# yisol/IDM-VTON

Hardware: AMD Instinct MI355X
Metric: try-on images/sec at 768x1024, 30 DDIM steps, guidance 2.0 (higher is better)
Workload: dtype bf16; 1 GPU; BASELINE.json configs[1]: 768x1024, 30 steps, batch 2/GPU, guidance 2.0, bf16 storage / fp32 accumulate, scheduler ddim, hipGraph on, GarmentNet batched over 6 timesteps, GarmentNet(block b+1)||TryonNet(block b) two-stream overlap on; images_per_call=2, parallelism=dp1 (image shards, one start-up RCCL weight broadcast), rccl_ranks=1

## Files before the change

idm-vton_amd/csrc/gemm_body.cuh:

```cuda
#pragma once
#include <type_traits>
#if !defined(__gfx950__) && !defined(__gfx942__) && defined(__HIP_DEVICE_COMPILE__)
#error "gemm_body.cuh: the counted vmcnt pipeline is written for gfx94x/gfx950 (stores counted in vmcnt)"
#endif
#include "common.cuh"
#include "gemm_common.cuh"

template <typename T, int BN, int BM, int WN, int WM, int ST, bool V1, bool LIN, bool PF, bool TR, bool XA = false>
__device__ __forceinline__ void gemm_body(const GemmParams& p, char* smem, const int m0, const int n0) {
    typedef typename VT<T>::v8 v8;
    typedef typename VT<T>::v4 v4;
    constexpr int NW = WN * WM;
    constexpr int SN = BN / WN, SM = BM / WM;
    constexpr int NI = SN / 32, MI = SM / 32;
    constexpr int WBYTES = BN * 128, XBYTES = BM * 128;
    constexpr int PW_ = BN / 8, PX_ = BM / 8;
    constexpr bool UNEVEN = (PW_ % NW != 0) || (PX_ % NW != 0);
    constexpr int WI = (PW_ + NW - 1) / NW, XI = (PX_ + NW - 1) / NW;
    static_assert(BN % 8 == 0 && BM % 8 == 0 && WN * SN == BN && WM * SM == BM && NI * 32 == SN && MI * 32 == SM, "tile / wave-count mismatch");
    static_assert(!UNEVEN || (V1 && ST == 2), "round-robin piece assignment needs the two-stage ring");
    char* sW = smem;
    char* sX = smem + ST * WBYTES;

    const int lane = threadIdx.x & 63;
// ... 110 lines not shown
    for (int ni = 0; ni < NI; ++ni)
#pragma unroll
        for (int mi = 0; mi < MI; ++mi)
#pragma unroll
            for (int r = 0; r < 16; ++r) acc[ni][mi][r] = 0.f;

    auto frag_a = [&](const char* bW, int s, int ni) { return *(const v8*)(bW + a_row[ni] + (((2 * s + u) ^ a_swz[ni]) << 4)); };
    auto frag_b = [&](const char* bX, int s, int mi) { return *(const v8*)(bX + b_row[mi] + (((2 * s + u) ^ b_swz[mi]) << 4)); };
    auto compute = [&](int buf, bool spread = false, int t_next = 0, int buf_next = 0) {
        const char* bW = sW + buf * WBYTES;
        const char* bX = sX + buf * XBYTES;
        if constexpr (!PF) {
#pragma unroll
            for (int s = 0; s < 4; ++s) {
                v8 a[NI], b[MI];
#pragma unroll
                for (int ni = 0; ni < NI; ++ni) a[ni] = frag_a(bW, s, ni);
#pragma unroll
                for (int mi = 0; mi < MI; ++mi) b[mi] = frag_b(bX, s, mi);
                if constexpr (V1) {
                    if (spread) issue_part(t_next, buf_next, s);
                    __builtin_amdgcn_sched_barrier(0);
                }
#pragma unroll
                for (int ni = 0; ni < NI; ++ni)
#pragma unroll
                    for (int mi = 0; mi < MI; ++mi)
                        acc[ni][mi] = TR ? VT<T>::mfma(b[mi], a[ni], acc[ni][mi]) : VT<T>::mfma(a[ni], b[mi], acc[ni][mi]);
            }
        } else {
            v8 a[2][NI], b[2][MI];
#pragma unroll
            for (int ni = 0; ni < NI; ++ni) a[0][ni] = frag_a(bW, 0, ni);
#pragma unroll
            for (int mi = 0; mi < MI; ++mi) b[0][mi] = frag_b(bX, 0, mi);
#pragma unroll
            for (int s = 0; s < 4; ++s) {
                if (s < 3) {
#pragma unroll
                    for (int ni = 0; ni < NI; ++ni) a[(s + 1) & 1][ni] = frag_a(bW, s + 1, ni);
#pragma unroll
                    for (int mi = 0; mi < MI; ++mi) b[(s + 1) & 1][mi] = frag_b(bX, s + 1, mi);
                }
                if (spread) issue_part(t_next, buf_next, s);
                __builtin_amdgcn_sched_barrier(0);
#pragma unroll
                for (int ni = 0; ni < NI; ++ni)
#pragma unroll
                    for (int mi = 0; mi < MI; ++mi)
                        acc[ni][mi] = TR ? VT<T>::mfma(b[s & 1][mi], a[s & 1][ni], acc[ni][mi])
                                         : VT<T>::mfma(a[s & 1][ni], b[s & 1][mi], acc[ni][mi]);
                __builtin_amdgcn_sched_barrier(0);
            }
        }
    };

    v8 xkf[XA ? XA_NK : 1];
    int xa_b = 0, xa_h = 0;
    if constexpr (XA) {
        static_assert(NI == 2 && !TR, "fused cross-attention: one 64-channel head per wave");
        const int mw = m0 + wm * SM;
        xa_b = (mw < p.M ? mw : p.M - 1) / p.xa.tokens;
        xa_h = (n0 + wn * SN) >> 6;
        xattn_load_k<T>(p.xa, xa_b, xa_h, lane, xkf);
    }
    const int nt = p.Ktot >> 6;
    if constexpr (!V1) {
        issue(0, 0);
        for (int t = 0; t < nt; ++t) {
            asm volatile("s_waitcnt vmcnt(0)" ::: "memory");
            __syncthreads();
            if (t + 1 < nt) issue(t + 1, (t + 1) & 1);
            compute(t & 1);
        }
    } else {
        constexpr int LPT = WI + XI;
        static_assert((ST - 2) * LPT < 64, "vmcnt immediate is 6 bits");
#pragma unroll
        for (int s = 0; s < ST - 1; ++s)
            if (s < nt) issue(s, s);
        int cbuf = 0, ibuf = ST - 1;
        for (int t = 0; t < nt; ++t) {
            if (t + ST - 2 < nt) wait_vmcnt<(ST - 2) * LPT>(); else wait_vmcnt<0>();
            __builtin_amdgcn_s_barrier();
            asm volatile("" ::: "memory");
            compute(cbuf, t + ST - 1 < nt, t + ST - 1, ibuf);
            cbuf = cbuf + 1 == ST ? 0 : cbuf + 1;
            ibuf = ibuf + 1 == ST ? 0 : ibuf + 1;
        }
    }

    if constexpr (XA) {
        v8 xvf[XA_NV];
        xattn_load_v<T>(p.xa, xa_b, xa_h, lane, xvf);
        xattn_compute<T, MI>(p.xa, p.M, acc, m0 + wm * SM, lane, xkf, xvf);
    }
    gemm_epilogue<T, NI, MI, SN, SM, TR>(p, acc, m0, n0, wn, wm, lane);
}

template <typename T, int BN, int BM, int WN, int WM, int ST, bool V1, bool LIN, int OCC, bool PFX = false>
__global__ __launch_bounds__(WN * WM * 64, OCC) void gemm_conv_kernel(const GemmParams p) {
    __shared__ __attribute__((aligned(1024))) char smem[ST * (BN + BM) * 128];
    const int wg = xcd_remap(blockIdx.x, p.tiles_m * p.tiles_n);
    int tm, tn;
    if constexpr (!V1) { tm = wg / p.tiles_n; tn = wg - tm * p.tiles_n; }
    else {
        const int GM = p.gm > 0 ? p.gm : 1024 / BM;
        const int width = GM * p.tiles_n;
        const int grp = wg / width, rem = wg - grp * width;
        const int first = grp * GM;
        const int gsz = p.tiles_m - first < GM ? p.tiles_m - first : GM;
        tn = rem / gsz; tm = first + (rem - tn * gsz);
    }
    const int m0 = tm * BM, n0 = tn * BN;
    if constexpr (BN == 320) {
        gemm_body<T, BN, BM, WN, WM, ST, V1, LIN, OCC == 1 || PFX, false>(p, smem, m0, n0);
    } else {
        if (p.vt != nullptr && n0 >= p.vt_n0) gemm_body<T, BN, BM, WN, WM, ST, V1, LIN, OCC == 1 || PFX, true>(p, smem, m0, n0);
        else gemm_body<T, BN, BM, WN, WM, ST, V1, LIN, OCC == 1 || PFX, false>(p, smem, m0, n0);
    }
}

template <typename T, int BN, int BM, int WN, int WM, int ST, int OCC>
__global__ __launch_bounds__(WN * WM * 64, OCC) void gemm_xattn_kernel(const GemmParams p) {
    __shared__ __attribute__((aligned(1024))) char smem[ST * (BN + BM) * 128];
    const int wg = xcd_remap(blockIdx.x, p.tiles_m * p.tiles_n);
    const int GM = p.gm > 0 ? p.gm : 1024 / BM;
    const int width = GM * p.tiles_n;
    const int grp = wg / width, rem = wg - grp * width;
    const int first = grp * GM;
    const int gsz = p.tiles_m - first < GM ? p.tiles_m - first : GM;
    const int tn = rem / gsz, tm = first + (rem - tn * gsz);
    gemm_body<T, BN, BM, WN, WM, ST, true, true, OCC == 1, false, true>(p, smem, tm * BM, tn * BN);
}

template <typename T, int BN, int BM, int WN, int WM, int ST, bool V1, int OCC, bool PFX = false>
static void launch_cfg(const GemmParams& p0, bool lin, hipStream_t st) {
    GemmParams p = p0;
    p.gm = V1 ? idmvton_choose_gm(p.tiles_m, p.tiles_n, BM, BN, p.Ktot) : 0;
    const dim3 grid(p.tiles_n * p.tiles_m), block(WN * WM * 64);
    if constexpr (V1) {
        if (lin) { hipLaunchKernelGGL((gemm_conv_kernel<T, BN, BM, WN, WM, ST, true, true, OCC, PFX>), grid, block, 0, st, p); return; }
    }
    hipLaunchKernelGGL((gemm_conv_kernel<T, BN, BM, WN, WM, ST, V1, false, OCC, PFX>), grid, block, 0, st, p);
}


int gemm_tiles_v0(const GemmParams& p, bool bf16, int bn, int bm, bool lin, hipStream_t st);
int gemm_tiles_v1(const GemmParams& p, bool bf16, int bn, int bm, bool lin, hipStream_t st);
int gemm_tiles_v2(const GemmParams& p, bool bf16, int bn, int bm, bool lin, hipStream_t st);
int gemm_tiles_w8(const GemmParams& p, bool bf16, int bn, int bm, int form, bool lin, hipStream_t st);
int gemm_tiles_xattn(const GemmParams& p, bool bf16, int bn, int bm, int w8, hipStream_t st);
int launch_gemm_lin(const GemmParams& p, bool bf16, int bm, int form, int grid_cap, hipStream_t st);
```

idm-vton_amd/csrc/gemm_conv.hip:

```cpp
#include <cstdlib>
#include <cstring>
#include <vector>
#include "gemm_body.cuh"

int launch_gemm_lin(const GemmParams& p, bool bf16, int bm, int form, int grid_cap, hipStream_t st);

#include <map>
#include <mutex>
#include <tuple>
int idmvton_choose_gm(int tiles_m, int tiles_n, int bm, int bn, int K) {
    static const char* env = getenv("IDMVTON_GM");
    if (env) return atoi(env);
    static const bool model = getenv("IDMVTON_GM_MODEL") && atoi(getenv("IDMVTON_GM_MODEL")) != 0;
    if (!model) return 0;
    static std::mutex mu;
    static std::map<std::tuple<int, int, int, int, int>, int> cache;
    const auto key = std::make_tuple(tiles_m, tiles_n, bm, bn, K);
    std::lock_guard<std::mutex> lk(mu);
    auto it = cache.find(key);
    if (it != cache.end()) return it->second;
    const int T = tiles_m * tiles_n, q = T / 8, r = T % 8;
    static const long cap = getenv("IDMVTON_GM_CAP_KB") ? atol(getenv("IDMVTON_GM_CAP_KB")) << 10 : (2l << 20);
    long best = -1; int best_gm = 0;
    for (int gm = 1; gm <= tiles_m; ++gm) {
        if (gm > 1 && (long)gm * bm * K * 2 > cap) break;
        long cost = 0;
        for (int x = 0; x < 8; ++x) {
            const int lo = x < r ? x * (q + 1) : r * (q + 1) + (x - r) * q, n = x < r ? q + 1 : q;
            int m_lo = tiles_m, m_hi = -1;
            std::vector<char> ms(tiles_m, 0), ns(tiles_n, 0);
            int cm = 0, cn = 0;
            for (int wg = lo; wg < lo + n; ++wg) {
                const int width = gm * tiles_n, grp = wg / width, rem = wg - grp * width, first = grp * gm;
                const int gsz = tiles_m - first < gm ? tiles_m - first : gm;
                const int tn = rem / gsz, tm = first + (rem - tn * gsz);
                if (!ms[tm]) { ms[tm] = 1; ++cm; }
                if (!ns[tn]) { ns[tn] = 1; ++cn; }
            }
            (void)m_lo; (void)m_hi;
            cost += (long)cm * bm + (long)cn * bn;
        }
        if (best < 0 || cost < best) { best = cost; best_gm = gm; }
    }
    cache[key] = best_gm;
    return best_gm;
}

static int launch_gemm(const GemmParams& p0, bool bf16, int variant, int bn, int bm, bool lin, hipStream_t st) {
    GemmParams p = p0;
    int form = 0;
    int grid_cap = 0;
    if (variant == 5) { form = bm & 15; grid_cap = (bm & 0x4000) ? 5 : 0; bm &= ~(15 | 0x4000); }
    p.tiles_n = (p.N + bn - 1) / bn;
    p.tiles_m = (p.M + bm - 1) / bm;
    int rc = 1;
    if (p.mode == IDMVTON_EPI_XATTN) {
        if (bm != 64 && p.xa.tokens % 64 != 0) {
            bm = 64;
            p.tiles_m = (p.M + bm - 1) / bm;
        }
        if (gemm_tiles_xattn(p, bf16, bn, bm, variant == 6 && bn == 128 && bm == 128, st))
            return idmvton_set_error(IDMVTON_E_ARG, "gemm_conv: IDMVTON_EPI_XATTN runs on the 128x64, 128x128 and 128x256 tiles (got %dx%d)", bn, bm);
        CHECK_LAUNCH("gemm_conv");
        return IDMVTON_OK;
    }
    if (variant == 0) rc = gemm_tiles_v0(p, bf16, bn, bm, lin, st);
    else if (variant == 1) rc = gemm_tiles_v1(p, bf16, bn, bm, lin, st);
    else if (variant == 2) rc = gemm_tiles_v2(p, bf16, bn, bm, lin, st);
    else if (variant == 5) {
        if (!(bn == 256 && (bm == 256 || bm == 192))) return idmvton_set_error(IDMVTON_E_ARG, "gemm_conv: variant 5 is the 256x256 / 256x192 tile");
        if (lin) rc = launch_gemm_lin(p, bf16, bm, form, grid_cap, st);
        else if (bm == 256) rc = gemm_tiles_v1(p, bf16, 256, 256, lin, st);
        else {
            p.tiles_n = (p.N + 127) / 128; p.tiles_m = (p.M + 255) / 256;
            rc = gemm_tiles_v1(p, bf16, 128, 256, lin, st);
        }
    } else if (variant == 6) {
        const int form6 = bm & 15;
        bm &= ~15;
        p.tiles_m = (p.M + bm - 1) / bm;
        if (bn == 320 && (p.vt || !p.wide || p.out8 || p.mode == IDMVTON_EPI_GEGLU)) {
            const int fbn = bn == 320 ? 128 : bn, fbm = bn == 320 ? 256 : bm;
            p.tiles_n = (p.N + fbn - 1) / fbn;
            p.tiles_m = (p.M + fbm - 1) / fbm;
            rc = gemm_tiles_v1(p, bf16, fbn, fbm, lin, st);
        } else rc = gemm_tiles_w8(p, bf16, bn, bm, form6, lin, st);
    } else return idmvton_set_error(IDMVTON_E_ARG, "gemm_conv: unknown variant %d", variant);
    if (rc) return idmvton_set_error(IDMVTON_E_ARG, "gemm_conv: variant %d has no %dx%d tile", variant, bn, bm);
    CHECK_LAUNCH("gemm_conv");
    return IDMVTON_OK;
}

extern "C" int idmvton_gemm_conv(const idmvton_gemm_conv_args* a, void* stream) {
    CHECK_ARG(a != nullptr, IDMVTON_E_ARG, "gemm_conv: null args");
    CHECK_ARG(a->dtype == IDMVTON_F16 || a->dtype == IDMVTON_BF16, IDMVTON_E_DTYPE, "gemm_conv: dtype %d", a->dtype);
    CHECK_ARG(a->M > 0 && a->N > 0 && a->Ktot > 0, IDMVTON_E_SHAPE, "gemm_conv: M=%d N=%d K=%d", a->M, a->N, a->Ktot);
    CHECK_ARG(a->Ktot % 64 == 0, IDMVTON_E_SHAPE, "gemm_conv: Ktot=%d must be a multiple of 64", a->Ktot);
    CHECK_ARG(a->N % 4 == 0, IDMVTON_E_SHAPE, "gemm_conv: N=%d must be a multiple of 4", a->N);
    CHECK_ARG(a->nseg >= 1 && a->nseg <= IDMVTON_MAX_SEG, IDMVTON_E_SHAPE, "gemm_conv: nseg=%d", a->nseg);
    int ksum = 0;
    for (int s = 0; s < a->nseg; ++s) {
        const idmvton_seg& g = a->seg[s];
        CHECK_ARG(g.ptr && g.len > 0 && g.len % 64 == 0, IDMVTON_E_SHAPE, "gemm_conv: seg %d len=%d", s, g.len);
        CHECK_ARG(g.pitch % 8 == 0 && g.coff % 8 == 0, IDMVTON_E_ALIGN, "gemm_conv: seg %d pitch=%d coff=%d", s, g.pitch, g.coff);
        CHECK_ARG(g.bytes < 0x80000000u, IDMVTON_E_SHAPE, "gemm_conv: seg %d tensor >= 2 GiB", s);
        CHECK_ARG(((uintptr_t)g.ptr & 15) == 0, IDMVTON_E_ALIGN, "gemm_conv: seg %d pointer not 16-byte aligned", s);
        ksum += g.len;
    }
    CHECK_ARG(ksum == a->Ktot, IDMVTON_E_SHAPE, "gemm_conv: segment lengths sum to %d, Ktot=%d", ksum, a->Ktot);
    CHECK_ARG(a->Ho > 0 && a->Wo > 0 && a->Hi > 0 && a->Wi > 0 && a->stride > 0 && a->M % (a->Ho * a->Wo) == 0,
              IDMVTON_E_SHAPE, "gemm_conv: geometry M=%d Ho=%d Wo=%d", a->M, a->Ho, a->Wo);
    if (a->ups) CHECK_ARG(a->stride == 1 && a->Ho <= 2 * a->Hi && a->Ho >= 2 * a->Hi - 1 && a->Wo <= 2 * a->Wi && a->Wo >= 2 * a->Wi - 1, IDMVTON_E_SHAPE,
                          "gemm_conv: ups=1 needs stride 1 and an output grid of 2Hi x 2Wi or one short of it (Ho=%d Hi=%d Wo=%d Wi=%d)", a->Ho, a->Hi, a->Wo, a->Wi);
    CHECK_ARG(a->w && ((uintptr_t)a->w & 15) == 0, IDMVTON_E_ALIGN, "gemm_conv: weight pointer");
    const uint64_t wbytes = (uint64_t)a->N * a->Ktot * 2;
    CHECK_ARG(wbytes + (uint64_t)128 * a->Ktot * 2 < 0xFFFFFFFFull, IDMVTON_E_SHAPE, "gemm_conv: weight too large");
    const bool geglu = a->mode == IDMVTON_EPI_GEGLU, xattn = a->mode == IDMVTON_EPI_XATTN;
    CHECK_ARG(a->mode == IDMVTON_EPI_NONE || a->mode == IDMVTON_EPI_GELU || a->mode == IDMVTON_EPI_QUICKGELU || geglu || xattn, IDMVTON_E_ARG, "gemm_conv: mode %d", a->mode);
    CHECK_ARG(a->colscale_n >= 0 && a->colscale_n % 4 == 0 && !(geglu && a->colscale_n), IDMVTON_E_ARG, "gemm_conv: colscale_n=%d", a->colscale_n);
    if (geglu) CHECK_ARG(a->N % 64 == 0 && !a->res && !a->rowbias && !a->vt, IDMVTON_E_ARG, "gemm_conv: GEGLU needs N%%64==0, no res/rowbias/vt");
    CHECK_ARG(a->out || (a->vt && a->vt_n0 == 0), IDMVTON_E_ARG, "gemm_conv: null out");
    if (a->out) CHECK_ARG(a->ldo % 4 == 0 && ((uintptr_t)a->out & 7) == 0, IDMVTON_E_ALIGN, "gemm_conv: out alignment");
    if (a->res) CHECK_ARG(a->ldr % 4 == 0 && ((uintptr_t)a->res & 7) == 0, IDMVTON_E_ALIGN, "gemm_conv: res alignment");
    if (a->bias) CHECK_ARG(((uintptr_t)a->bias & 7) == 0, IDMVTON_E_ALIGN, "gemm_conv: bias alignment");
    if (a->rowbias) CHECK_ARG(a->rowbias_ld % 4 == 0 && a->rows_per_group > 0 && ((uintptr_t)a->rowbias & 7) == 0,
                              IDMVTON_E_ALIGN, "gemm_conv: rowbias");
    if (a->vt && a->vt_perm) CHECK_ARG(((uintptr_t)a->vt & 15) == 0, IDMVTON_E_ALIGN, "gemm_conv: vt pointer not 16-byte aligned");
    if (a->vt && a->vt_perm) CHECK_ARG(a->vt_tokens % 16 == 0, IDMVTON_E_ARG, "gemm_conv: vt_perm needs vt_tokens %% 16 == 0 (got %d)", a->vt_tokens);
    if (a->vt) CHECK_ARG(a->vt_tokens > 0 && a->vt_tokens % 4 == 0 && a->M % a->vt_tokens == 0 && a->vt_n0 % 64 == 0 &&
                         a->vt_n0 >= 0 && a->vt_n0 < a->N && ((uintptr_t)a->vt & 7) == 0,
                         IDMVTON_E_ARG, "gemm_conv: vt_tokens=%d vt_n0=%d", a->vt_tokens, a->vt_n0);

    GemmParams p;
    memset(&p.xa, 0, sizeof(p.xa));
    if (xattn) {
        const idmvton_xattn* x = a->xattn;
        CHECK_ARG(x != nullptr && (x->nseg == 1 || x->nseg == 2), IDMVTON_E_ARG, "gemm_conv: IDMVTON_EPI_XATTN needs `xattn` with 1 or 2 key segments");
        CHECK_ARG(a->N % 64 == 0 && !a->bias && !a->res && !a->rowbias && !a->vt && !a->colscale_n && !a->io_flags &&
                  a->nseg == 1 && a->Ho == 1 && a->Hi == 1 && a->Wo == a->M && a->Wi == a->M && a->out && a->ldo % 8 == 0 && ((uintptr_t)a->out & 15) == 0,
                  IDMVTON_E_ARG, "gemm_conv: IDMVTON_EPI_XATTN is a plain Linear with N %% 64 == 0 and nothing else in its epilogue");
        CHECK_ARG(x->tokens > 0 && x->tokens % 32 == 0 && a->M % x->tokens == 0, IDMVTON_E_SHAPE, "gemm_conv: xattn.tokens=%d (rows per batch element, a multiple of 32 dividing M=%d)", x->tokens, a->M);
        for (int s = 0; s < x->nseg; ++s) {
            const int nk_max = s == 0 ? 96 : 32;
            CHECK_ARG(x->k[s] && x->vt[s] && x->nk[s] > 0 && x->nk[s] <= nk_max && x->k_rows[s] >= ((x->nk[s] + 31) & ~31) && x->ldk[s] >= a->N && x->ldk[s] % 8 == 0 &&
                      x->ldvt[s] >= ((x->nk[s] + 15) & ~15) && x->ldvt[s] % 8 == 0 && (((uintptr_t)x->k[s] | (uintptr_t)x->vt[s]) & 15) == 0, IDMVTON_E_SHAPE,
                      "gemm_conv: xattn segment %d: nk=%d (<= %d) k_rows=%d (>= round32(nk)) ldk=%d ldvt=%d (>= round16(nk))", s, x->nk[s], nk_max, x->k_rows[s], x->ldk[s], x->ldvt[s]);
            p.xa.k[s] = x->k[s]; p.xa.vt[s] = x->vt[s]; p.xa.ldk[s] = x->ldk[s]; p.xa.ldvt[s] = x->ldvt[s]; p.xa.nk[s] = x->nk[s]; p.xa.krows[s] = x->k_rows[s];
        }
        p.xa.nseg = x->nseg; p.xa.tokens = x->tokens; p.xa.vchan = a->N; p.xa.ip_scale = x->ip_scale;
    } else CHECK_ARG(a->xattn == nullptr, IDMVTON_E_ARG, "gemm_conv: `xattn` without mode IDMVTON_EPI_XATTN");
    p.w = a->w; p.w_bytes = (uint32_t)wbytes; p.N = a->N; p.Ktot = a->Ktot;
    p.nseg = a->nseg;
    for (int s = 0; s < IDMVTON_MAX_SEG; ++s) p.seg[s] = a->seg[s < a->nseg ? s : a->nseg - 1];
    p.M = a->M; p.Ho = a->Ho; p.Wo = a->Wo; p.Hi = a->Hi; p.Wi = a->Wi; p.stride = a->stride; p.ups = a->ups ? 1 : 0;
    p.out = a->out; p.ldo = a->ldo; p.bias = a->bias; p.rowbias = a->rowbias; p.rowbias_ld = a->rowbias_ld;
    p.rows_per_group = a->rows_per_group > 0 ? a->rows_per_group : 1; p.res = a->res; p.ldr = a->ldr; p.mode = a->mode;
    p.vt = a->vt; p.vt_n0 = a->vt_n0; p.vt_tokens = a->vt_tokens > 0 ? a->vt_tokens : 4; p.vt_perm = a->vt_perm ? 1 : 0;
    p.colscale_n = a->colscale_n; p.colscale = a->colscale;
    p.tiles_m = p.tiles_n = 0; p.gm = 0;
    {
        auto a16 = [](const void* q) { return ((uintptr_t)q & 15) == 0; };
        const int n_out = geglu ? a->N / 2 : a->N;
        p.wide = n_out % 8 == 0 && a->N % 8 == 0 && a->colscale_n % 8 == 0 && (!a->out || (a->ldo % 8 == 0 && a16(a->out))) &&
                 (!a->res || (a->ldr % 8 == 0 && a16(a->res))) && (!a->bias || a16(a->bias)) &&
                 (!a->rowbias || (a->rowbias_ld % 8 == 0 && a16(a->rowbias))) && (!a->vt || a->vt_n0 % 8 == 0);
    }

    int variant = 1, bn = 64, bm = 64;
    static const bool env_narrow = getenv("IDMVTON_EPILOGUE_8B") != nullptr;
    if ((a->tile_hint & 0x8000) || env_narrow) p.wide = 0;
    p.res32 = (a->io_flags & IDMVTON_IO_RES_F32) ? 1 : 0;
    p.out32 = (a->io_flags & IDMVTON_IO_OUT_F32) ? 1 : 0;
    p.bias32 = (a->io_flags & IDMVTON_IO_BIAS_F32) ? 1 : 0;
    if (p.bias32) CHECK_ARG(a->bias && p.wide && !geglu && !a->vt && ((uintptr_t)a->bias & 15) == 0, IDMVTON_E_ARG,
                            "gemm_conv: IDMVTON_IO_BIAS_F32 needs a 16-byte aligned bias and the plain 16-byte epilogue (no GEGLU, no vt)");
    CHECK_ARG((a->io_flags & ~15) == 0, IDMVTON_E_ARG, "gemm_conv: io_flags=%d", a->io_flags);
    p.out8 = (a->io_flags & IDMVTON_IO_OUT_F8) ? 1 : 0;
    p.o8_scale = a->f8_out_scale; p.vt8_scale = a->f8_vt_scale;
    if (p.out8) {
        CHECK_ARG(a->io_flags == IDMVTON_IO_OUT_F8 && a->mode == IDMVTON_EPI_NONE && !a->res && !a->rowbias && p.wide,
                  IDMVTON_E_ARG, "gemm_conv: IDMVTON_IO_OUT_F8 needs the plain 16-byte epilogue (no activation / residual / rowbias / fp32 IO)");
        CHECK_ARG((!a->out || a->f8_out_scale > 0.f) && (!a->vt || (a->f8_vt_scale > 0.f && a->vt_tokens % 64 == 0 && ((uintptr_t)a->vt & 15) == 0)),
                  IDMVTON_E_ARG, "gemm_conv: IDMVTON_IO_OUT_F8: scales > 0, vt_tokens %% 64 == 0 (got %d), 16-byte aligned vt", a->vt_tokens);
    }
    if (p.res32 || p.out32) {
        CHECK_ARG((a->io_flags & ~7) == 0 && !geglu && !a->vt, IDMVTON_E_ARG, "gemm_conv: io_flags=%d (fp32 res / out: no GEGLU, no vt)", a->io_flags);
        CHECK_ARG(!p.res32 || a->res, IDMVTON_E_ARG, "gemm_conv: IDMVTON_IO_RES_F32 without res");
        CHECK_ARG(p.wide, IDMVTON_E_ALIGN, "gemm_conv: the fp32 residual stream needs the 16-byte epilogue (N, ldo, ldr multiples of 8, 16-byte aligned pointers)");
    }
    if (a->tile_hint) { variant = (a->tile_hint >> 28) & 0xf; bn = (a->tile_hint >> 16) & 0xfff; bm = a->tile_hint & 0x7fff; }
    else {
        static const int cand[5][2] = {{256, 256}, {128, 256}, {128, 128}, {128, 64}, {64, 64}};
        for (int i = 0; i < 5; ++i) {
            const int n_ = cand[i][0], m_ = cand[i][1];
            if (geglu && n_ < 128) continue;
            if (xattn && (n_ != 128)) continue;
            if (a->vt && a->vt_n0 % n_ != 0) continue;
            if (i < 4 && (n_ > ((a->N + 63) & ~63) || m_ > ((a->M + 63) & ~63))) continue;
            bn = n_; bm = m_;
            if ((long)((a->N + n_ - 1) / n_) * ((a->M + m_ - 1) / m_) >= 200) break;
        }
    }
    if (geglu) CHECK_ARG(bn >= 128, IDMVTON_E_ARG, "gemm_conv: GEGLU needs BN >= 128 (64-row wave tiles)");
    if (a->vt) CHECK_ARG(a->vt_n0 % bn == 0, IDMVTON_E_ARG, "gemm_conv: vt_n0 %% BN != 0");
    const idmvton_seg& s0 = a->seg[0];
    const bool lin = a->nseg == 1 && a->Ho == 1 && a->Hi == 1 && a->Wo == a->M && a->Wi == a->M && a->stride == 1 &&
                     !a->ups && s0.dy == 0 && s0.dx == 0 && (uint64_t)a->M * s0.pitch * 2 < 0x80000000ull;
    if (!a->tile_hint && bn == 256 && bm == 256 && lin) { variant = 5; bm = 257; }
    else if (!a->tile_hint && !xattn) {
        if (bn == 256 && bm == 256) variant = 6;
        else if (bn == 128 && bm == 128) variant = 6;
        if (a->N > 256 && a->N <= 320 && p.wide && !a->vt && !geglu && !p.out8 && (a->M + 191) / 192 >= 200) { variant = 6; bn = 320; bm = 192; }
    }
    hipStream_t st = (hipStream_t)stream;
    return launch_gemm(p, a->dtype == IDMVTON_BF16, variant, bn, bm, lin, st);
}
```

idm-vton_amd/ops.py:

```python
import ctypes as C
import json
import os

import torch

from . import ffi

_DT = {torch.float16: ffi.F16, torch.bfloat16: ffi.BF16}


def _dt(t):
    try:
        return _DT[t.dtype]
    except KeyError:
        raise TypeError(f"idm_vton_amd ops take float16/bfloat16 tensors, got {t.dtype}") from None


def _stream():
    return torch.cuda.current_stream().cuda_stream


PROFILE = None


def _call(fn_name, args, flops=0.0, bytes_=0.0, seg_nb=None):
    launch = (lambda: ffi.call(fn_name, args, _stream())) if seg_nb is None else (lambda: ffi.call_shared(fn_name, args, seg_nb, _stream()))
    if PROFILE is None:
        launch()
        return
    e0, e1 = torch.cuda.Event(enable_timing=True), torch.cuda.Event(enable_timing=True)
    e0.record()
    launch()
    e1.record()
    PROFILE.append((fn_name, e0, e1, flops, bytes_))


TUNE_PATH = os.environ.get("IDMVTON_TUNE_TABLE") or os.path.join(os.path.dirname(os.path.abspath(__file__)), "tune_gfx950.json")
_TUNE = {"gemm": {}, "attn": {}}
RECORD = None


def load_tune(path=TUNE_PATH):
    global _TUNE
    _TUNE = {"gemm": {}, "attn": {}}
    if path and os.path.exists(path):
        with open(path) as f:
            t = json.load(f)
        _TUNE = {"gemm": dict(t.get("gemm", {})), "attn": dict(t.get("attn", {}))}
        for kind in ("gemm", "attn") if os.environ.get("IDMVTON_TUNE_NO_MIRROR") != "1" else ():
            for k, v in list(_TUNE[kind].items()):
                d, rest = k.split(",", 1)
                if d in ("0", "1"):
                    _TUNE[kind].setdefault(("1" if d == "0" else "0") + "," + rest, v)
    return _TUNE


def gemm_key(a):
    return "%d,%d,%d,%d,%d,%d,%d,%d,%d,%d" % (a.dtype, a.M, a.N, a.Ktot, a.nseg, a.Wo, a.stride, a.ups, a.mode, 1 if a.vt else 0)


def attn_key(a):
    return "%d,%d,%d,%d,%d,%d,%d,%d,%d" % (a.dtype, a.mode, a.B, a.heads, a.Nq, a.nseg, a.nk[0], a.nk[1] if a.nseg > 1 else 0,
                                          a.seg_b0[1] if a.nseg > 1 else 0)


def _dev(t):
    if not t.is_cuda:
        raise RuntimeError("idm_vton_amd ops run on the GPU only (tensor is on %s); there is no CPU fallback" % t.device)
    return t


def _ptr(t):
    return None if t is None else _dev(t).data_ptr()


class SegSpec:
    __slots__ = ("t", "coff", "len", "dy", "dx")

    def __init__(self, t, coff, length, dy=0, dx=0):
        self.t, self.coff, self.len, self.dy, self.dx = t, coff, length, dy, dx


def gemm_conv(segs, w, M, *, Ho=1, Wo=None, Hi=1, Wi=None, stride=1, ups=False, out=None, ldo=None, bias=None,
              rowbias=None, rowbias_ld=0, rows_per_group=1, res=None, ldr=None, geglu=False, gelu=False, quick_gelu=False, vt=None,
              vt_n0=0, vt_tokens=0, vt_perm=True, colscale_n=0, colscale=1.0, tile_hint=0, out_f32=False, xattn=None, f8=None):
    if f8 is not None:
        if res is not None or rowbias is not None or geglu or gelu or quick_gelu or (bias is not None and bias.dtype == torch.float32):
            raise ValueError("gemm_conv(f8=...): no residual / rowbias / activation, and the bias in the storage dtype (not fp32)")
        if vt is not None and vt_tokens % 64 != 0:
            raise ValueError(f"gemm_conv(f8=...): vt_tokens must be a multiple of 64 (got {vt_tokens})")
    a = ffi.GemmConvArgs()
    a.dtype = _dt(w)
    N, Ktot = w.shape
    a.w, a.N, a.Ktot = _ptr(w), N, Ktot
    a.nseg = len(segs)
    for i, s in enumerate(segs):
        t = _dev(s.t)
        g = a.seg[i]
        pitch = t.shape[-1]
        for d in range(t.dim() - 2, -1, -1):
            if t.shape[d] > 1:
                pitch = t.stride(d)
                break
        extent = 1 + sum((n - 1) * st for n, st in zip(t.shape, t.stride()))
        g.ptr, g.bytes, g.pitch = t.data_ptr(), extent * t.element_size(), pitch
        g.coff, g.len, g.dy, g.dx = s.coff, s.len, s.dy, s.dx
    Wo = M if Wo is None else Wo
    Wi = M if Wi is None else Wi
    a.M, a.Ho, a.Wo, a.Hi, a.Wi, a.stride, a.ups = M, Ho, Wo, Hi, Wi, stride, int(bool(ups))
    n_out = N // 2 if geglu else (vt_n0 if vt is not None else N)
    if out is None and n_out > 0:
        out = torch.empty((M, n_out), dtype=torch.uint8 if f8 is not None else (torch.float32 if out_f32 else w.dtype), device=w.device)
    if f8 is not None:
        if (out is not None and out.dtype != torch.uint8) or (vt is not None and vt.dtype != torch.uint8):
            raise TypeError("gemm_conv(f8=...): out / vt must be uint8 (e4m3 bytes)")
        a.f8_out_scale, a.f8_vt_scale = float(f8[0]), float(f8[1])
    a.io_flags = ffi.IO_OUT_F8 if f8 is not None else (
        (ffi.IO_RES_F32 if res is not None and res.dtype == torch.float32 else 0) |
        (ffi.IO_OUT_F32 if out is not None and out.dtype == torch.float32 else 0) |
        (ffi.IO_BIAS_F32 if bias is not None and bias.dtype == torch.float32 else 0))
    a.out = _ptr(out)
    a.ldo = (ldo if ldo is not None else (out.stride(-2) if out is not None else 0))
    a.bias = _ptr(bias)
    a.rowbias, a.rowbias_ld, a.rows_per_group = _ptr(rowbias), rowbias_ld, rows_per_group
    a.res = _ptr(res)
    a.ldr = (ldr if ldr is not None else (res.stride(-2) if res is not None else 0))
    a.mode = ffi.EPI_GEGLU if geglu else (ffi.EPI_GELU if gelu else (ffi.EPI_QUICKGELU if quick_gelu else ffi.EPI_NONE))
    xa, xflops = None, 0.0
    if xattn is not None:
        xa = ffi.XAttn()
        xa.nseg, xa.tokens, xa.ip_scale = len(xattn["segs"]), xattn["tokens"], xattn.get("ip_scale", 1.0)
        for i, sg in enumerate(xattn["segs"]):
            xa.k[i], xa.vt[i], xa.ldk[i], xa.ldvt[i], xa.nk[i], xa.k_rows[i] = _ptr(sg["k"]), _ptr(sg["vt"]), sg["ldk"], sg["ldvt"], sg["nk"], sg["k_rows"]
            xflops += 4.0 * M * N * sg["nk"]
        a.mode, a.xattn = ffi.EPI_XATTN, C.pointer(xa)
    a.vt, a.vt_n0, a.vt_tokens = _ptr(vt), vt_n0, vt_tokens
    a.vt_perm = int(bool(vt_perm)) if vt is not None else 0
    a.colscale_n, a.colscale = colscale_n, colscale
    a.tile_hint = tile_hint if tile_hint else _TUNE["gemm"].get(gemm_key(a), 0)
    if RECORD is not None:
        RECORD.append(("gemm", gemm_key(a), type(a).from_buffer_copy(a), (segs, w, out, bias, rowbias, res, vt, xa, xattn)))
    seen, xbytes = set(), 0
    for sg in segs:
        if sg.t.data_ptr() not in seen:
            seen.add(sg.t.data_ptr())
            xbytes += sg.t.numel() * sg.t.element_size()
    esz = w.element_size()
    obytes = (M * (N // 2 if geglu else N)) * (out.element_size() if out is not None else esz) + (M * N * res.element_size() if res is not None else 0)
    _call("idmvton_gemm_conv", a, flops=2.0 * M * N * Ktot + xflops, bytes_=float(xbytes + N * Ktot * esz + obytes))
    return out


def xattn_q_weight(w):
    return w.index_select(0, key_order_index(w.shape[0], w.device)).contiguous()


def key_order_index(n, device=None):
    if n % 16:
        raise ValueError("key order needs a multiple of 16 keys, got %d" % n)
    i = torch.arange(n, device=device)
    return (i & ~12) | ((i & 4) << 1) | ((i & 8) >> 1)


def key_order(vt):
    return vt.index_select(-1, key_order_index(vt.shape[-1], vt.device)).contiguous()


def round16(n):
    return (n + 15) // 16 * 16


def linear(x, w, **kw):
    M, K = x.shape
    return gemm_conv([SegSpec(x, 0, K)], w, M, **kw)


def conv_segs(x, k, pad, coff=0, length=None):
    length = x.shape[-1] if length is None else length
    return [SegSpec(x, coff, length, ky - pad, kx - pad) for ky in range(k) for kx in range(k)]


QSCALE = 0.125 * 1.4426950408889634


def attention(q, out, segs, heads, *, mode=ffi.ATTN_SELF, ip_scale=1.0, B=None, Nq=None, ldq=None, ldo=None, tune=0, q_prescaled=False):
    a = ffi.AttnArgs()
    a.dtype, a.mode = _dt(q), mode
    a.B = q.shape[0] if B is None else B
    a.Nq = q.shape[1] if Nq is None else Nq
    a.heads = heads
    a.q, a.ldq = _ptr(q), (q.stride(-2) if ldq is None else ldq)
    a.out, a.ldo = _ptr(out), (out.stride(-2) if ldo is None else ldo)
    a.nseg = len(segs)
    for i, s in enumerate(segs):
        a.k[i], a.vt[i] = _ptr(s["k"]), _ptr(s["vt"])
        a.ldk[i], a.ldvt[i] = s["ldk"], s["ldvt"]
        a.nk[i], a.k_rows[i], a.seg_b0[i] = s["nk"], s.get("k_rows", 0), s.get("b0", 0)
    a.ip_scale = ip_scale
    a.q_prescaled = int(bool(q_prescaled))
    a.tune = tune
    if not tune:
        t = _TUNE["attn"].get(attn_key(a), 0)
        a.tune = t if (q_prescaled or ((t >> 16) & 0xff) not in (7, 8, 16)) else 0
    if RECORD is not None:
        RECORD.append(("attn", attn_key(a), type(a).from_buffer_copy(a), (q, out, segs)))
    fl = 0.0
    for s in segs:
        fl += 4.0 * (a.B - s.get("b0", 0)) * heads * a.Nq * s["nk"] * 64
    nb = _seg_nb(segs)
    _call("idmvton_attn_fwd_shared" if nb else "idmvton_attn_fwd", a, flops=fl, bytes_=2.0 * a.B * a.Nq * heads * 64 * q.element_size(), seg_nb=nb)
    return out


def _seg_nb(segs):
    nb = [int(s.get("nb", 0) or 0) for s in segs] + [0] * (2 - len(segs))
    return nb if any(nb) else None


def quant_f8(src, scale, mode=0, out=None):
    rows, cols = src.shape
    ldd = cols if mode == 0 else (cols + 63) // 64 * 64
    if out is None:
        out = torch.empty((rows, ldd), dtype=torch.uint8, device=src.device)
    a = ffi.QuantF8Args()
    a.dtype, a.mode, a.rows, a.cols = _dt(src), mode, rows, cols
    a.src, a.lds, a.dst, a.ldd, a.scale = _ptr(src), src.stride(0), _ptr(out), out.stride(0), scale
    _call("idmvton_quant_f8", a, bytes_=float(rows * cols * (src.element_size() + 1)))
    return out


def attention_f8(q8, out, segs, heads, *, qk_scale_exp, v_scale_exp, B, Nq, ldq=None, ldo=None):
    a = ffi.AttnF8Args()
    a.out_dtype, a.B, a.heads, a.Nq = _dt(out), B, heads, Nq
    a.q8, a.ldq = _ptr(q8), (q8.stride(-2) if ldq is None else ldq)
    a.out, a.ldo = _ptr(out), (out.stride(-2) if ldo is None else ldo)
    a.nseg = len(segs)
    fl = 0.0
    for i, s in enumerate(segs):
        a.k8[i], a.vt8[i] = _ptr(s["k8"]), _ptr(s["vt8"])
        a.ldk[i], a.ldvt[i] = s["ldk"], s["ldvt"]
        a.nk[i], a.k_rows[i], a.seg_b0[i] = s["nk"], s.get("k_rows", 0), s.get("b0", 0)
        fl += 4.0 * (B - s.get("b0", 0)) * heads * Nq * s["nk"] * 64
    a.qk_scale_exp, a.v_scale_exp = qk_scale_exp, v_scale_exp
    nb = _seg_nb(segs)
    _call("idmvton_attn_f8_shared" if nb else "idmvton_attn_f8", a, flops=fl, bytes_=float(B * Nq * heads * 64 * (1 + out.element_size())), seg_nb=nb)
    return out


def attention_small(q, k, v, out, heads, d, *, scale, causal=False, B=None, Lq=None, Lk=None, ldq=None, ldk=None, ldv=None, ldo=None):
    a = ffi.AttnSmallArgs()
    a.dtype = _dt(q)
    a.B = q.shape[0] if B is None else B
    a.heads, a.d = heads, d
    a.Lq = q.shape[1] if Lq is None else Lq
    a.Lk = k.shape[1] if Lk is None else Lk
    a.q, a.ldq = _ptr(q), (q.stride(-2) if ldq is None else ldq)
    a.k, a.ldk = _ptr(k), (k.stride(-2) if ldk is None else ldk)
    a.v, a.ldv = _ptr(v), (v.stride(-2) if ldv is None else ldv)
    a.out, a.ldo = _ptr(out), (out.stride(-2) if ldo is None else ldo)
    a.scale, a.causal = scale, int(bool(causal))
    _call("idmvton_attn_small", a, flops=4.0 * a.B * heads * a.Lq * a.Lk * d)
    return out


def layernorm(x, gamma, beta, eps=1e-5, out=None, out2=None):
    rows, Cc = x.shape
    if out is None:
        out = torch.empty((rows, Cc), dtype=gamma.dtype, device=x.device)
    a = ffi.LayerNormArgs()
    a.dtype, a.rows, a.C = _dt(gamma), rows, Cc
    a.x_f32 = int(x.dtype == torch.float32)
    a.x, a.ldx = _ptr(x), x.stride(0)
    a.gamma, a.beta, a.eps = _ptr(gamma), _ptr(beta), eps
    a.y, a.ldy = _ptr(out), out.stride(0)
    a.y2, a.ldy2 = _ptr(out2), (out2.stride(0) if out2 is not None else 0)
    _call("idmvton_layernorm", a, bytes_=(x.element_size() + (1.0 + (out2 is not None)) * out.element_size()) * rows * Cc)
    return out


def groupnorm(x, gamma, beta, groups, eps, silu, stats, x2=None, out=None, split_dtype=None):
    B, HW, C1 = x.shape
    Cc = C1 + (x2.shape[-1] if x2 is not None else 0)
    prec = split_dtype is not None
    if prec and not (x.dtype == gamma.dtype == beta.dtype == torch.float32 and (x2 is None or x2.dtype == torch.float32)):
        raise TypeError("groupnorm(split_dtype=...): x, gamma and beta must be float32")
    if out is None:
        out = torch.empty((B, HW, 2 * Cc if prec else Cc), dtype=split_dtype if prec else x.dtype, device=x.device)
    a = ffi.GroupNormArgs()
    a.dtype, a.B, a.HW, a.C, a.groups = _dt(out), B, HW, Cc, groups
    a.flags = (ffi.GN_X_F32 | ffi.GN_Y_SPLIT | ffi.GN_AFFINE_F32) if prec else 0
    a.x, a.C1, a.x2 = _ptr(x), C1, _ptr(x2)
    a.gamma, a.beta, a.eps, a.silu = _ptr(gamma), _ptr(beta), eps, int(bool(silu))
# ... 110 lines not shown
```

Baseline: 1.580 images/s.

## Add halo-tile implicit-GEMM kernel for stride-1 3x3 convolutions

Measured after the change: 1.607 images/s (median of 6 runs). +1.7%, better.

```diff
diff --git a/idm-vton_amd/csrc/gemm_body.cuh b/idm-vton_amd/csrc/gemm_body.cuh
--- a/idm-vton_amd/csrc/gemm_body.cuh
+++ b/idm-vton_amd/csrc/gemm_body.cuh
@@ -286,3 +286,6 @@
 int gemm_tiles_w8(const GemmParams& p, bool bf16, int bn, int bm, int form, bool lin, hipStream_t st);
 int gemm_tiles_xattn(const GemmParams& p, bool bf16, int bn, int bm, int w8, hipStream_t st);
 int launch_gemm_lin(const GemmParams& p, bool bf16, int bm, int form, int grid_cap, hipStream_t st);
+int gemm_tiles_halo(const GemmParams& p, bool bf16, int bn, int bm, hipStream_t st);
+int idmvton_halo_route(const GemmParams& p);
+int idmvton_halo_rows(int H, int W, int bm);
diff --git a/idm-vton_amd/csrc/gemm_conv.hip b/idm-vton_amd/csrc/gemm_conv.hip
--- a/idm-vton_amd/csrc/gemm_conv.hip
+++ b/idm-vton_amd/csrc/gemm_conv.hip
@@ -85,6 +85,10 @@
             p.tiles_m = (p.M + fbm - 1) / fbm;
             rc = gemm_tiles_v1(p, bf16, fbn, fbm, lin, st);
         } else rc = gemm_tiles_w8(p, bf16, bn, bm, form6, lin, st);
+    } else if (variant == 7) {
+        rc = gemm_tiles_halo(p, bf16, bn, bm, st);
+        if (rc == 2) return idmvton_set_error(IDMVTON_E_ARG, "gemm_conv: variant 7 runs stride-1 3x3 convolutions (9 tap segments over one tensor, then centre-tap "
+                                              "segments; no upsample / V^T part) whose halo patch fits the %dx%d tile (H=%d W=%d)", bn, bm, p.Hi, p.Wi);
     } else return idmvton_set_error(IDMVTON_E_ARG, "gemm_conv: unknown variant %d", variant);
     if (rc) return idmvton_set_error(IDMVTON_E_ARG, "gemm_conv: variant %d has no %dx%d tile", variant, bn, bm);
     CHECK_LAUNCH("gemm_conv");
@@ -212,6 +216,11 @@
         else if (bn == 128 && bm == 128) variant = 6;
         if (a->N > 256 && a->N <= 320 && p.wide && !a->vt && !geglu && !p.out8 && (a->M + 191) / 192 >= 200) { variant = 6; bn = 320; bm = 192; }
     }
+    if (!a->tile_hint && !xattn) {
+        static const bool halo_off = getenv("IDMVTON_HALO_OFF") != nullptr;
+        const int hb = halo_off ? 0 : idmvton_halo_route(p);
+        if (hb) { variant = 7; bn = hb >> 16; bm = hb & 0xffff; }
+    }
     hipStream_t st = (hipStream_t)stream;
     return launch_gemm(p, a->dtype == IDMVTON_BF16, variant, bn, bm, lin, st);
 }
diff --git a/idm-vton_amd/csrc/gemm_tiles_halo.hip b/idm-vton_amd/csrc/gemm_tiles_halo.hip
--- /dev/null
+++ b/idm-vton_amd/csrc/gemm_tiles_halo.hip
@@ -0,0 +1,239 @@
+#include "gemm_body.cuh"
+
+int idmvton_halo_rows(int H, int W, int bm) {
+    const long HW = (long)H * W, PW = W + 2, PHW = (long)(H + 2) * PW;
+    auto q = [&](long m) { const long b = m / HW, rem = m - b * HW, y = rem / W, x = rem - y * W; return b * PHW + (y + 1) * PW + x + 1; };
+    long a = bm, b = HW;
+    while (b) { const long t = a % b; a = b; b = t; }
+    long worst = 0;
+    for (long r = 0; r < HW; r += a) {
+        const long span = q(r + bm - 1) - q(r) + 2 * PW + 3;
+        if (span > worst) worst = span;
+    }
+    return (int)worst;
+}
+
+template <typename T, int BN, int BM, int WN, int WM, int HP>
+__global__ __launch_bounds__(WN * WM * 64, 2) void gemm_halo_kernel(const GemmParams p) {
+    typedef typename VT<T>::v8 v8;
+    constexpr int NW = WN * WM, ST = 3;
+    constexpr int SN = BN / WN, SM = BM / WM, NI = SN / 32, MI = SM / 32;
+    constexpr int WBYTES = BN * 128, HROWS = HP * NW * 8, HBYTES = HROWS * 128;
+    constexpr int WI = BN / 8 / NW, XB = BM / 8 / NW;
+    static_assert(WI * NW * 8 == BN && XB * NW * 8 == BM && WN * SN == BN && WM * SM == BM && NI * 32 == SN && MI * 32 == SM, "tile / wave-count mismatch");
+    static_assert(WI >= 1 && WI <= 3 && XB >= 1 && XB <= HP && HP <= 8, "DMA pieces are dealt over the four k-steps / the taps 0..7");
+    static_assert(ST * WBYTES + 2 * HBYTES <= 160 * 1024, "LDS budget");
+    __shared__ __attribute__((aligned(1024))) char smem[ST * WBYTES + 2 * HBYTES];
+    char* sW = smem;
+    char* sH = smem + ST * WBYTES;
+
+    const int wg = xcd_remap(blockIdx.x, p.tiles_m * p.tiles_n);
+    int tm, tn;
+    {
+        const int GM = p.gm > 0 ? p.gm : 1024 / BM;
+        const int width = GM * p.tiles_n;
+        const int grp = wg / width, rem = wg - grp * width;
+        const int first = grp * GM;
+        const int gsz = p.tiles_m - first < GM ? p.tiles_m - first : GM;
+        tn = rem / gsz; tm = first + (rem - tn * gsz);
+    }
+    const int m0 = tm * BM, n0 = tn * BN;
+
+    const int lane = threadIdx.x & 63;
+    const int wave = uniform(threadIdx.x >> 6);
+    const int wn = wave / WM, wm = wave % WM;
+    const int u = lane >> 5, l31 = lane & 31;
+    const int lrow = lane >> 3, lslot = lane & 7;
+
+    const idmvton_seg sg0 = p.seg[0];
+    const int Cin = sg0.len;
+    const int S = Cin >> 6;
+    const int nt = p.Ktot >> 6;
+    const int H = p.Hi, W = p.Wi, HW = H * W, PW = W + 2, PHW = (H + 2) * PW;
+    auto qof = [&](int m) { const int b = m / HW, rem = m - b * HW, y = rem / W, x = rem - y * W; return b * PHW + (y + 1) * PW + x + 1; };
+    const int q0 = qof(m0);
+    const int m_last = m0 + BM - 1 < p.M ? m0 + BM - 1 : p.M - 1;
+    const int q_lo = q0 - PW - 1;
+    const int need = qof(m_last) - q0 + 2 * PW + 3;
+    const int nimg = p.M / HW;
+
+    uint32_t w_off[WI];
+#pragma unroll
+    for (int i = 0; i < WI; ++i) {
+        const int R = (wave * WI + i) * 8 + lrow;
+        const int c = lslot ^ ((R >> 1) & 7);
+        w_off[i] = ((uint32_t)(n0 + R) * (uint32_t)p.Ktot + c * 8) * 2u;
+    }
+    uint32_t h_off[HP];
+#pragma unroll
+    for (int i = 0; i < HP; ++i) {
+        const int h = (wave * HP + i) * 8 + lrow;
+        const int c = lslot ^ ((h >> 1) & 7);
+        const int qh = q_lo + h;
+        const int b = qh / PHW, rem = qh - b * PHW;
+        const int py = rem / PW, px = rem - py * PW;
+        const bool ok = h < need && b < nimg && py >= 1 && py <= H && px >= 1 && px <= W;
+        h_off[i] = ok ? ((uint32_t)(b * HW + (py - 1) * W + (px - 1)) * (uint32_t)sg0.pitch + sg0.coff + c * 8) * 2u : OOB_SENTINEL;
+    }
+    int b_m[XB], b_c8[XB];
+#pragma unroll
+    for (int i = 0; i < XB; ++i) {
+        const int R = (wave * XB + i) * 8 + lrow;
+        b_m[i] = m0 + R < p.M ? m0 + R : -1;
+        b_c8[i] = (lslot ^ ((R >> 1) & 7)) * 8;
+    }
+    const __amdgpu_buffer_rsrc_t rs_w = make_rsrc(p.w, p.w_bytes);
+    const __amdgpu_buffer_rsrc_t rs_x0 = make_rsrc(sg0.ptr, sg0.bytes);
+    int bsi = 9 < IDMVTON_MAX_SEG ? 9 : IDMVTON_MAX_SEG - 1, bks = 0;
+    idmvton_seg sgb = p.seg[bsi];
+    __amdgpu_buffer_rsrc_t rs_b = make_rsrc(sgb.ptr, sgb.bytes);
+    auto advance_b = [&]() {
+        bks += 64;
+        if (bks >= sgb.len) {
+            bks = 0;
+            bsi = bsi + 1 < IDMVTON_MAX_SEG ? bsi + 1 : IDMVTON_MAX_SEG - 1;
+            sgb = p.seg[bsi];
+            rs_b = make_rsrc(sgb.ptr, sgb.bytes);
+        }
+    };
+
+    auto koff = [&](int t) -> uint32_t {
+        if (t >= 9 * S) return (uint32_t)t * 64u;
+        const int s = t / 9, tap = t - 9 * s;
+        return (uint32_t)(tap * Cin + s * 64);
+    };
+    auto issue_w = [&](int t, int i) { dma16(rs_w, sW + (t % ST) * WBYTES + (wave * WI + i) * 1024, w_off[i] + koff(t) * 2u); };
+    auto issue_x = [&](int n, int i) {
+        char* d = sH + (n & 1) * HBYTES;
+        if (n < S) dma16(rs_x0, d + (wave * HP + i) * 1024, h_off[i] + (uint32_t)n * 128u);
+        else if (i < XB) {
+            const uint32_t off = ((uint32_t)b_m[i] * (uint32_t)sgb.pitch + sgb.coff + bks + b_c8[i]) * 2u;
+            dma16(rs_b, d + (wave * XB + i) * 1024, (8 * S + n < nt && b_m[i] >= 0) ? off : OOB_SENTINEL);
+        } else dma16(rs_x0, d + (BM / 8 + wave * (HP - XB) + (i - XB)) * 1024, OOB_SENTINEL);
+    };
+
+    int a_row[NI], a_swz[NI], d_q[MI], d_lin[MI];
+#pragma unroll
+    for (int ni = 0; ni < NI; ++ni) { const int r = wn * SN + ni * 32 + l31; a_row[ni] = r * 128; a_swz[ni] = (r >> 1) & 7; }
+#pragma unroll
+    for (int mi = 0; mi < MI; ++mi) {
+        const int r = wm * SM + mi * 32 + l31;
+        const int m = m0 + r < p.M ? m0 + r : p.M - 1;
+        d_q[mi] = qof(m) - q0;
+        d_lin[mi] = r;
+    }
+
+    f32x16 acc[NI][MI];
+#pragma unroll
+    for (int ni = 0; ni < NI; ++ni)
+#pragma unroll
+        for (int mi = 0; mi < MI; ++mi)
+#pragma unroll
+            for (int r = 0; r < 16; ++r) acc[ni][mi][r] = 0.f;
+
+    auto compute = [&](const char* bW, const char* bX, const int (&x_row)[MI], auto&& parts) {
+        int xr[MI], xs[MI];
+#pragma unroll
+        for (int mi = 0; mi < MI; ++mi) { xr[mi] = x_row[mi] * 128; xs[mi] = (x_row[mi] >> 1) & 7; }
+#pragma unroll
+        for (int ks = 0; ks < 4; ++ks) {
+            v8 a[NI], b[MI];
+#pragma unroll
+            for (int ni = 0; ni < NI; ++ni) a[ni] = *(const v8*)(bW + a_row[ni] + (((2 * ks + u) ^ a_swz[ni]) << 4));
+#pragma unroll
+            for (int mi = 0; mi < MI; ++mi) b[mi] = *(const v8*)(bX + xr[mi] + (((2 * ks + u) ^ xs[mi]) << 4));
+            parts(ks);
+            __builtin_amdgcn_sched_barrier(0);
+#pragma unroll
+            for (int ni = 0; ni < NI; ++ni)
+#pragma unroll
+                for (int mi = 0; mi < MI; ++mi) acc[ni][mi] = VT<T>::mfma(a[ni], b[mi], acc[ni][mi]);
+        }
+    };
+
+#pragma unroll
+    for (int i = 0; i < HP; ++i) issue_x(0, i);
+#pragma unroll
+    for (int i = 0; i < WI; ++i) issue_w(0, i);
+#pragma unroll
+    for (int i = 0; i < WI; ++i) issue_w(1, i);
+
+    int t = 0;
+    for (int s = 0; s < S; ++s) {
+        const char* bH = sH + (s & 1) * HBYTES;
+#pragma unroll
+        for (int tap = 0; tap < 9; ++tap, ++t) {
+            if (t + 1 < nt) { if (tap >= 1 && tap - 1 < HP) wait_vmcnt<WI + 1>(); else wait_vmcnt<WI>(); }
+            else wait_vmcnt<0>();
+            __builtin_amdgcn_s_barrier();
+            asm volatile("" ::: "memory");
+            const int toff = (tap / 3) * PW + tap % 3;
+            int x_row[MI];
+#pragma unroll
+            for (int mi = 0; mi < MI; ++mi) x_row[mi] = d_q[mi] + toff;
+            compute(sW + (t % ST) * WBYTES, bH, x_row, [&](int ks) {
+                if (ks == 0) { if (tap < HP) issue_x(s + 1, tap); }
+                else if (ks - 1 < WI && t + 2 < nt) issue_w(t + 2, ks - 1);
+            });
+        }
+        if (s + 1 >= S) advance_b();
+    }
+    for (int n = S; t < nt; ++t, ++n) {
+        if (t + 1 < nt) wait_vmcnt<WI>(); else wait_vmcnt<0>();
+        __builtin_amdgcn_s_barrier();
+        asm volatile("" ::: "memory");
+        compute(sW + (t % ST) * WBYTES, sH + (n & 1) * HBYTES, d_lin, [&](int ks) {
+            if (ks == 0) {
+#pragma unroll
+                for (int i = 0; i < XB; ++i) issue_x(n + 1, i);
+            } else if (ks - 1 < WI && t + 2 < nt) issue_w(t + 2, ks - 1);
+        });
+        advance_b();
+    }
+    gemm_epilogue<T, NI, MI, SN, SM, false>(p, acc, m0, n0, wn, wm, lane);
+}
+
+static bool halo_pattern(const GemmParams& p) {
+    if (p.nseg < 9 || p.stride != 1 || p.ups || p.Ho != p.Hi || p.Wo != p.Wi || p.vt || p.mode == IDMVTON_EPI_XATTN || p.mode == IDMVTON_EPI_GEGLU) return false;
+    const idmvton_seg& a = p.seg[0];
+    for (int s = 0; s < 9; ++s) {
+        const idmvton_seg& g = p.seg[s];
+        if (g.ptr != a.ptr || g.bytes != a.bytes || g.pitch != a.pitch || g.coff != a.coff || g.len != a.len || g.dy != s / 3 - 1 || g.dx != s % 3 - 1) return false;
+    }
+    for (int s = 9; s < p.nseg; ++s)
+        if (p.seg[s].dy != 0 || p.seg[s].dx != 0) return false;
+    return true;
+}
+
+template <typename T, int BN, int BM, int WN, int WM, int HP>
+static int launch_halo(const GemmParams& p0, hipStream_t st) {
+    if (idmvton_halo_rows(p0.Hi, p0.Wi, BM) > HP * WN * WM * 8) return 2;
+    GemmParams p = p0;
+    p.tiles_n = (p.N + BN - 1) / BN;
+    p.tiles_m = (p.M + BM - 1) / BM;
+    p.gm = idmvton_choose_gm(p.tiles_m, p.tiles_n, BM, BN, p.Ktot);
+    hipLaunchKernelGGL((gemm_halo_kernel<T, BN, BM, WN, WM, HP>), dim3(p.tiles_n * p.tiles_m), dim3(WN * WM * 64), 0, st, p);
+    return 0;
+}
+
+template <typename T>
+static int run(const GemmParams& p, int bn, int bm, hipStream_t st) {
+    if (bn == 128 && bm == 128) return launch_halo<T, 128, 128, 2, 4, 6>(p, st);
+    if (bn == 128 && bm == 256) return launch_halo<T, 128, 256, 2, 4, 6>(p, st);
+    if (bn == 64 && bm == 64) return launch_halo<T, 64, 64, 2, 2, 6>(p, st);
+    return 1;
+}
+
+int gemm_tiles_halo(const GemmParams& p, bool bf16, int bn, int bm, hipStream_t st) {
+    if (!halo_pattern(p)) return 2;
+    return bf16 ? run<bf16_t>(p, bn, bm, st) : run<f16_t>(p, bn, bm, st);
+}
+
+int idmvton_halo_route(const GemmParams& p) {
+    if (!halo_pattern(p) || p.Wi > 64 || p.seg[0].len < 320) return 0;
+    if (idmvton_halo_rows(p.Hi, p.Wi, 128) > 384) return 0;
+    const long tn = (p.N + 127) / 128;
+    if (idmvton_halo_rows(p.Hi, p.Wi, 256) <= 384 && tn * ((p.M + 255) / 256) >= 200) return (128 << 16) | 256;
+    if (tn * ((p.M + 127) / 128) >= 200 || idmvton_halo_rows(p.Hi, p.Wi, 64) > 192) return (128 << 16) | 128;
+    return (64 << 16) | 64;
+}
diff --git a/idm-vton_amd/ops.py b/idm-vton_amd/ops.py
--- a/idm-vton_amd/ops.py
+++ b/idm-vton_amd/ops.py
@@ -1,5 +1,7 @@
 import ctypes as C
+import functools
 import json
+import math
 import os
 
 import torch
@@ -62,6 +64,48 @@
 def attn_key(a):
     return "%d,%d,%d,%d,%d,%d,%d,%d,%d" % (a.dtype, a.mode, a.B, a.heads, a.Nq, a.nseg, a.nk[0], a.nk[1] if a.nseg > 1 else 0,
                                           a.seg_b0[1] if a.nseg > 1 else 0)
+
+
+HALO_OFF = os.environ.get("IDMVTON_HALO_OFF") is not None
+HALO_CAP = {(128, 128): 384, (128, 256): 384, (64, 64): 192}
+
+
+def halo_q(m, H, W):
+    b, rem = divmod(m, H * W)
+    y, x = divmod(rem, W)
+    return b * (H + 2) * (W + 2) + (y + 1) * (W + 2) + x + 1
+
+
+@functools.lru_cache(maxsize=None)
+def halo_rows(H, W, bm):
+    return max(halo_q(r + bm - 1, H, W) - halo_q(r, H, W) for r in range(0, H * W, math.gcd(bm, H * W))) + 2 * (W + 2) + 3
+
+
+def halo_pattern(segs, Ho, Wo, Hi, Wi, stride, ups, vt, xattn):
+    if len(segs) < 9 or stride != 1 or ups or Ho != Hi or Wo != Wi or vt is not None or xattn is not None:
+        return False
+    a = segs[0]
+    for i, g in enumerate(segs):
+        if i < 9:
+            if g.t is not a.t or g.coff != a.coff or g.len != a.len or (g.dy, g.dx) != (i // 3 - 1, i % 3 - 1):
+                return False
+        elif g.dy or g.dx:
+            return False
+    return True
+
+
+def halo_routed(segs, Ho, Wo, Hi, Wi, stride, ups, vt=None, xattn=None):
+    return (not HALO_OFF and halo_pattern(segs, Ho, Wo, Hi, Wi, stride, ups, vt, xattn) and Wi <= 64 and segs[0].len >= 320
+            and halo_rows(Hi, Wi, 128) <= HALO_CAP[(128, 128)])
+
+
+def halo_tile(M, N, Hi, Wi):
+    tn = (N + 127) // 128
+    if halo_rows(Hi, Wi, 256) <= HALO_CAP[(128, 256)] and tn * ((M + 255) // 256) >= 200:
+        return 128, 256
+    if tn * ((M + 127) // 128) >= 200 or halo_rows(Hi, Wi, 64) > HALO_CAP[(64, 64)]:
+        return 128, 128
+    return 64, 64
 
 
 def _dev(t):
@@ -137,7 +181,12 @@
     a.vt, a.vt_n0, a.vt_tokens = _ptr(vt), vt_n0, vt_tokens
     a.vt_perm = int(bool(vt_perm)) if vt is not None else 0
     a.colscale_n, a.colscale = colscale_n, colscale
-    a.tile_hint = tile_hint if tile_hint else _TUNE["gemm"].get(gemm_key(a), 0)
+    if tile_hint:
+        a.tile_hint = tile_hint
+    elif not geglu and halo_routed(segs, Ho, Wo, Hi, Wi, stride, ups, vt, xattn):
+        a.tile_hint = 0
+    else:
+        a.tile_hint = _TUNE["gemm"].get(gemm_key(a), 0)
     if RECORD is not None:
         RECORD.append(("gemm", gemm_key(a), type(a).from_buffer_copy(a), (segs, w, out, bias, rowbias, res, vt, xa, xattn)))
     seen, xbytes = set(), 0
```
